# TimD1/vcfdist

Measured on AMD Instinct MI355X. Metric: supercluster-alignments/sec, higher is better.
Workload: dtype int32; 1 GPU; wgs_synth; superclusters_per_gpu=1000000, span_dist=lognormal(median 20, sigma 1.2) clip [4,10000]

## Files before the change

### vcfdist_amd/csrc/pr_zl.hip

```cpp
#ifndef PR_ZL_HIP_
#define PR_ZL_HIP_
#include <type_traits>


#define ZW_PTR(w) (int((w) & 0xffffu) - 1)
#define ZW_BASE(w) (((w) >> 16) & 0x7fu)
#define ZW_PV (1u << 23)
#define ZW_PB (1u << 24)
#define ZW_PE (1u << 25)
#define ZW_INS (1u << 26)
#define ZW_TP (1u << 27)
__device__ __forceinline__ bool zw_fwd_allow(uint32_t w) { return !(w & ZW_PV) || (w & ZW_PE); }
__device__ __forceinline__ bool zw_bwd_allow(uint32_t w) { return !(w & ZW_PV) || (w & ZW_PB); }

#define ZE_ALIVE 1u
#define ZE_HASMAT 2u
#define ZE_HASSWP 4u
#define ZE_PSLOT_SHIFT 3
#define ZE_TP 32u
#define ZE_BWD 64u

#define ZL_MAXLEN 65000
#define ZL_CLEAN_REJECT (-1)

__global__ void __launch_bounds__(256) k_prep_zl(DevBatch B, const AlnDesc *__restrict__ descs, const int32_t *__restrict__ list,
                                                 int n_list, const ZlWave *__restrict__ hdr, uint32_t *__restrict__ zin) {
    __shared__ uint32_t tile[64][65];
    __shared__ int64_t s_qo[64], s_ro[64], s_to[64];
    __shared__ int32_t s_lq[64], s_lr[64], s_lt[64];
    __shared__ uint8_t s_qs[64], s_ts[64];
    const int w = blockIdx.x;
    const ZlWave H = hdr[w];
    const int lane = threadIdx.x & 63, sub = threadIdx.x >> 6;
    if (threadIdx.x < 64) {
        const int wi = w * 64 + lane;
        const int a = wi < n_list ? list[wi] : -1;
        if (a >= 0) {
            const AlnDesc *d = descs + a;
            s_qo[lane] = d->q_off; s_ro[lane] = d->r_off; s_to[lane] = d->t_off;
            s_lq[lane] = d->Lq; s_lr[lane] = d->Lr; s_lt[lane] = d->Lt;
            s_qs[lane] = uint8_t(d->qs); s_ts[lane] = uint8_t(d->ts);
        } else {
            s_qo[lane] = s_ro[lane] = s_to[lane] = 0;
            s_lq[lane] = s_lr[lane] = s_lt[lane] = 0;
            s_qs[lane] = 0; s_ts[lane] = 2;
        }
    }
    __syncthreads();
    auto flagbits = [](int f) -> uint32_t { return ((f & PV) ? ZW_PV : 0u) | ((f & PB) ? ZW_PB : 0u) | ((f & PE) ? ZW_PE : 0u); };
    uint32_t *out = zin + H.in_off;
    for (int arr = 0; arr < 3; arr++) {
        const int mlen = arr == 0 ? H.mq : (arr == 1 ? H.mr : H.mt);
        for (int x0 = 0; x0 < mlen; x0 += 64) {
            const int x = x0 + lane;
#pragma unroll 16
            for (int k = 0; k < 16; k++) {
                const int l = sub * 16 + k;
                const int qs = s_qs[l], ts = s_ts[l];
                const int Lr = s_lr[l];
                const int len = arr == 0 ? s_lq[l] : (arr == 1 ? Lr : s_lt[l]);
                uint32_t v = 0x7f0000u;
                if (x < len) {
                    const int64_t ro = s_ro[l];
                    const int slot = arr == 2 ? ts : qs;
                    const int64_t o = (arr == 0 ? s_qo[l] : (arr == 1 ? ro : s_to[l])) + x;
                    const uint8_t *seq = arr == 1 ? B.ref_seq : B.hap_seq[slot];
                    const int2 *wk = arr == 0 ? B.wk_q[qs] : (arr == 1 ? B.wk_r[qs] : B.wk_t[ts - 2]);
                    const int2 k2 = wk[o];
                    const int p = k2.x, f = arr == 1 ? int(B.ref_flag[qs][o]) : (k2.y & 0xff);
                    const uint32_t ins = ((k2.y >> 8) & ((1 << qs) | (1 << ts))) ? ZW_INS : 0u;
                    v = uint32_t((p + 1) & 0xffff) | (uint32_t(seq[o] & 0x7f) << 16) | flagbits(f) | ins;
                    if (arr == 0 && x > 0 && ((p != wk[o - 1].x + 1) || (f & PB))) v |= ZW_TP;
                    (void)Lr;
                }
                tile[lane][l] = v;
            }
            __syncthreads();
            const int rows = min(64, mlen - x0);
            for (int r = sub; r < rows; r += 4) out[int64_t(x0 + r) * 64 + lane] = tile[r][lane];
            __syncthreads();
        }
        out += int64_t(mlen) * 64;
    }
}

typedef __attribute__((ext_vector_type(4))) unsigned int zl_u4;
typedef __attribute__((ext_vector_type(2))) unsigned int zl_u2;
#define ZL_OOB 0xfffffff0u

__global__ void __launch_bounds__(64, 6) k_zero_lane(const AlnDesc *__restrict__ descs, const int32_t *__restrict__ list, int n_list,
                                                  const ZlWave *__restrict__ hdr, const uint32_t *__restrict__ zin,
                                                  uint4 *__restrict__ zlog, AlnOut *__restrict__ outs, PathEnt *__restrict__ paths,
                                                  int keep_paths, int d1_max_rows, int prio_rows) {
    const int w = blockIdx.x, lane = threadIdx.x;
    const ZlWave H = hdr[w];
    if (H.mt >= prio_rows) __builtin_amdgcn_s_setprio(2);
    const int wi = w * 64 + lane;
    const int a_ = wi < n_list ? list[wi] : -1;
    const bool live = a_ >= 0;
    const int a = max(a_, 0);
    const AlnDesc *dp = descs + a;
    const int Lq = live ? dp->Lq : 1, Lr = live ? dp->Lr : 1, Lt = live ? dp->Lt : 0;
    const int L[2] = {Lq, Lr};
    const auto rin = __builtin_amdgcn_make_buffer_rsrc(const_cast<uint32_t *>(zin + H.in_off), 0, 256 * (H.mq + H.mr + H.mt), 0x00020000);
    const auto rlog = __builtin_amdgcn_make_buffer_rsrc(zlog + H.log_off, 0, 1280 * H.mt, 0x00020000);
    const uint32_t lane4 = uint32_t(lane) << 2, lane8 = uint32_t(lane) << 3;
    const uint32_t pos0[2] = {0u, uint32_t(H.mq) << 8}, post = uint32_t(H.mq + H.mr) << 8;
    const uint32_t logP0 = uint32_t(H.mt) << 9;
    auto in_at = [&](uint32_t off) -> uint32_t { return __builtin_amdgcn_raw_buffer_load_b32(rin, off, 0, 0); };
    bool ok = live && Lq < ZL_MAXLEN && Lr < ZL_MAXLEN && Lt < ZL_MAXLEN && Lt >= 2;
    const int rows = ok ? Lt : 0;
    int tmax = rows;
#pragma unroll
    for (int o = 32; o; o >>= 1) tmax = max(tmax, __shfl_xor(tmax, o));
    if (tmax == 0) {
        if (live) { outs[a].dist_q = D_INF; outs[a].dist_r = D_INF; outs[a].exit_min = 0; }
        return;
    }

    int qri[2][4];
    uint32_t pw[2][4];
#pragma unroll
    for (int p = 0; p < 2; p++) {
#pragma unroll
        for (int s = 0; s < 4; s++) { qri[p][s] = -1; pw[p][s] = 0; }
    }
    uint32_t tw0 = in_at(ok ? post + lane4 : ZL_OOB);
    if (ok) {
        qri[0][0] = 0; pw[0][0] = in_at(pos0[0] + lane4);
        qri[1][0] = 0; pw[1][0] = in_at(pos0[1] + lane4);
        zl_u2 e0;
        e0.x = ZE_ALIVE | ZE_HASMAT | ((pw[0][0] & ZW_TP) ? ZE_TP : 0u) | (zw_bwd_allow(pw[0][0]) ? ZE_BWD : 0u);
        e0.y = ZE_ALIVE | ZE_HASMAT | (zw_bwd_allow(pw[1][0]) ? ZE_BWD : 0u);
        __builtin_amdgcn_raw_buffer_store_b64(e0, rlog, lane8, 0, 0);
    }
    uint32_t pf_mw[2][2] = {{0, 0}, {0, 0}}, pf_sw[2][2] = {{0, 0}, {0, 0}};
    bool have_pf = false;
    auto fwd_row = [&](auto Sc, int t, bool act, uint32_t tw1) -> bool {
        constexpr int S = decltype(Sc)::value;
        const bool t_allow = zw_fwd_allow(tw0);
        uint32_t mw[2][S], sw[2][S];
        int sz[2][S];
        const bool use_pf = S == 2 && have_pf;
#pragma unroll
        for (int p = 0; p < 2; p++) {
#pragma unroll
            for (int s = 0; s < S; s++) {
                const bool alive = act && qri[p][s] >= 0;
                const int c = qri[p][s] + 1;
                const int z = ZW_PTR(pw[p][s]) + 1;
                const bool sok = alive && t_allow && zw_fwd_allow(pw[p][s]) && z < L[1 - p];
                sz[p][s] = sok ? z : -1;
                if (use_pf) {
                    mw[p][s] = (alive && c < L[p]) ? pf_mw[p][s & 1] : 0u;
                    sw[p][s] = sok ? pf_sw[p][s & 1] : 0u;
                } else {
                    mw[p][s] = in_at((alive && c < L[p]) ? pos0[p] + (uint32_t(c) << 8) + lane4 : ZL_OOB);
                    sw[p][s] = in_at(sok ? pos0[1 - p] + (uint32_t(z) << 8) + lane4 : ZL_OOB);
                }
            }
        }
        const uint32_t Tb = ZW_BASE(tw1);
        int nq[2][S];
        uint32_t nw[2][S], ne[2][S];
#pragma unroll
        for (int p = 0; p < 2; p++) {
#pragma unroll
            for (int s = 0; s < S; s++) {
                const bool hit = act && qri[p][s] >= 0 && ZW_BASE(mw[p][s]) == Tb;
                nq[p][s] = hit ? qri[p][s] + 1 : -1;
                nw[p][s] = mw[p][s];
                ne[p][s] = hit ? ZE_HASMAT : 0u;
            }
        }
        bool bad = false, full = false;
#pragma unroll
        for (int p = 0; p < 2; p++) {
            const int o = 1 - p;
#pragma unroll
            for (int s = 0; s < S; s++) {
                const bool hit = sz[p][s] >= 0 && ZW_BASE(sw[p][s]) == Tb;
                if (!__any(hit)) continue;
                const int z = sz[p][s];
                int at = -1;
#pragma unroll
                for (int k = S - 1; k >= 0; k--) at = (nq[o][k] < 0) ? k : at;
#pragma unroll
                for (int k = 0; k < S; k++) at = (nq[o][k] == z) ? k : at;
                full = full || (hit && at < 0);
#pragma unroll
                for (int k = 0; k < S; k++) {
                    const bool here = hit && at == k;
                    bad = bad || (here && (ne[o][k] & ZE_HASSWP));
                    nq[o][k] = here ? z : nq[o][k];
                    nw[o][k] = here ? sw[p][s] : nw[o][k];
                    ne[o][k] = here ? (ne[o][k] | ZE_HASSWP | (uint32_t(s) << ZE_PSLOT_SHIFT)) : ne[o][k];
                }
            }
        }
        if (S < 4 && __any(full)) return false;
        ok = ok && !bad && !full;
        if (S == 2) {
#pragma unroll
            for (int p = 0; p < 2; p++) {
#pragma unroll
                for (int s = 0; s < 2; s++) {
                    const bool alive = act && ok && nq[p][s] >= 0;
                    const int c = nq[p][s] + 1;
                    const int z = ZW_PTR(nw[p][s]) + 1;
                    pf_mw[p][s] = in_at((alive && c < L[p]) ? pos0[p] + (uint32_t(c) << 8) + lane4 : ZL_OOB);
                    pf_sw[p][s] = in_at((alive && zw_fwd_allow(nw[p][s]) && z < L[1 - p]) ? pos0[1 - p] + (uint32_t(z) << 8) + lane4 : ZL_OOB);
                }
            }
        }
        have_pf = S == 2;
        {
            zl_u2 ev;
            uint32_t wq = 0, wr_ = 0;
#pragma unroll
            for (int sl = 0; sl < S; sl++) {
                wq |= (nq[0][sl] < 0 ? 0u : (ZE_ALIVE | ne[0][sl] | ((nw[0][sl] & ZW_TP) ? ZE_TP : 0u) | (zw_bwd_allow(nw[0][sl]) ? ZE_BWD : 0u))) << (8 * sl);
                wr_ |= (nq[1][sl] < 0 ? 0u : (ZE_ALIVE | ne[1][sl] | (zw_bwd_allow(nw[1][sl]) ? ZE_BWD : 0u))) << (8 * sl);
            }
            ev.x = wq; ev.y = wr_;
            __builtin_amdgcn_raw_buffer_store_b64(ev, rlog, (act && ok) ? (uint32_t(t + 1) << 9) + lane8 : ZL_OOB, 0, 0);
        }
#pragma unroll
        for (int p = 0; p < 2; p++) {
#pragma unroll
            for (int s = 0; s < S; s++) { qri[p][s] = act ? nq[p][s] : qri[p][s]; pw[p][s] = act ? nw[p][s] : pw[p][s]; }
        }
        tw0 = act ? tw1 : tw0;
        return true;
    };
    for (int t = 0; t + 1 < tmax; t++) {
        const bool act = ok && t + 1 < rows;
        const uint32_t tw1 = in_at(act ? post + (uint32_t(t + 1) << 8) + lane4 : ZL_OOB);
        bool upper = false;
#pragma unroll
        for (int p = 0; p < 2; p++) upper = upper || (act && (qri[p][2] >= 0 || qri[p][3] >= 0));
        if (__any(upper) || !fwd_row(std::integral_constant<int, 2>{}, t, act, tw1))
            (void)fwd_row(std::integral_constant<int, 4>{}, t, act, tw1);
    }
    int endq = -1, endr = -1;
#pragma unroll
    for (int s = 0; s < 4; s++) {
        if (qri[0][s] == Lq - 1) endq = s;
        if (qri[1][s] == Lr - 1) endr = s;
    }
    const bool clean = ok && Lt <= d1_max_rows;
    ok = ok && (endq >= 0 || endr >= 0);
    if (live) {
        AlnOut &o = outs[a];
        o.dist_q = (ok && endq >= 0) ? 0 : D_INF;
        o.dist_r = (ok && endr >= 0) ? 0 : D_INF;
        o.exit_min = ok ? D_INF : (clean ? ZL_CLEAN_REJECT : 0);
    }
    if (!__any(ok)) return;

    const int nrow = ok ? Lt : 0;
    int sc[2][4];
#pragma unroll
    for (int p = 0; p < 2; p++) {
#pragma unroll
        for (int s = 0; s < 4; s++) sc[p][s] = -1;
    }
    int bmax = nrow;
#pragma unroll
    for (int o = 32; o; o >>= 1) bmax = max(bmax, __shfl_xor(bmax, o));
    auto log_row = [&](int t, bool on) -> zl_u2 {
        return __builtin_amdgcn_raw_buffer_load_b64(rlog, on ? (uint32_t(t) << 9) + lane8 : ZL_OOB, 0, 0);
    };
    zl_u2 cur = zl_u2{0, 0};
    auto bwd_row = [&](auto Sc, int t, bool act, zl_u2 pre) {
        constexpr int S = decltype(Sc)::value;
        int best[2][S];
        uint32_t pp[2][S];
#pragma unroll
        for (int p = 0; p < 2; p++) {
#pragma unroll
            for (int s = 0; s < S; s++) { best[p][s] = -1; pp[p][s] = 0; }
        }
#pragma unroll
        for (int p = 0; p < 2; p++) {
            const int o = 1 - p;
#pragma unroll
            for (int s = 0; s < S; s++) {
                const bool on = act && sc[p][s] >= 0;
                const uint32_t e = ((p ? cur.y : cur.x) >> (8 * s)) & 0xffu;
                const int tp = (e & ZE_TP) ? 1 : 0;
                {
                    const bool m = on && (e & ZE_HASMAT);
                    const int v = sc[p][s] + tp;
                    const bool gt = m && v > best[p][s], eq = m && v == best[p][s];
                    best[p][s] = gt ? v : best[p][s];
                    pp[p][s] = gt ? 1u : (eq ? (pp[p][s] | 1u) : pp[p][s]);
                }
                {
                    const bool m = on && (e & ZE_HASSWP) && (e & ZE_BWD);
                    const int v = sc[p][s] + (p == 1 ? 0 : tp);
                    const int ps = int((e >> ZE_PSLOT_SHIFT) & 3u);
                    const uint32_t mine = 2u | (uint32_t(s) << 2);
#pragma unroll
                    for (int k = 0; k < S; k++) {
                        const bool h_ = m && ps == k;
                        const bool gt = h_ && v > best[o][k], eq = h_ && v == best[o][k];
                        best[o][k] = gt ? v : best[o][k];
                        pp[o][k] = gt ? mine : (eq ? ((pp[o][k] & 1u) | mine) : pp[o][k]);
                    }
                }
            }
        }
        uint32_t ppw = 0;
#pragma unroll
        for (int p = 0; p < 2; p++) {
#pragma unroll
            for (int s = 0; s < 4; s++) {
                if (s < S) {
                    ppw |= (best[p][s] >= 0 ? pp[p][s] : 0u) << (4 * (p * 4 + s));
                    sc[p][s] = act ? best[p][s] : sc[p][s];
                } else {
                    sc[p][s] = act ? -1 : sc[p][s];
                }
            }
        }
        __builtin_amdgcn_raw_buffer_store_b32(ppw, rlog, act ? logP0 + (uint32_t(t - 1) << 8) + lane4 : ZL_OOB, 0, 0);
        if (act) cur = pre;
    };
    auto row_at = [&](int r) -> zl_u2 { return log_row(r, r >= 0 && r < nrow); };
    zl_u2 lastpre = row_at(bmax - 1);
    zl_u2 rA = row_at(bmax - 2), rB = row_at(bmax - 3), rC = row_at(bmax - 4), rD = zl_u2{0, 0};
    auto bwd_step = [&](int t, const zl_u2 &pre_reg, zl_u2 &next_reg) {
        const bool act = t >= 1 && t < nrow;
        const bool first = t == nrow - 1 && t >= 1;
        if (first) {
            const int ep = endq >= 0 ? 0 : 1, es = endq >= 0 ? endq : endr;
            cur = lastpre;
#pragma unroll
            for (int p = 0; p < 2; p++) {
#pragma unroll
                for (int s = 0; s < 4; s++) sc[p][s] = (p == ep && s == es) ? 0 : -1;
            }
        }
        next_reg = row_at(t - 4);
        const zl_u2 pre = pre_reg;
        const bool upper = act && (((cur.x | cur.y | pre.x | pre.y) & 0xffff0000u) != 0u);
        if (__any(upper)) bwd_row(std::integral_constant<int, 4>{}, t, act, pre);
        else bwd_row(std::integral_constant<int, 2>{}, t, act, pre);
        lastpre = pre;
    };
    for (int t = bmax - 1; t >= 1; t -= 4) {
        bwd_step(t, rA, rD);
        bwd_step(t - 1, rB, rA);
        bwd_step(t - 2, rC, rB);
        bwd_step(t - 3, rD, rC);
    }
    const int beg_plane = sc[0][0] >= 0 ? VPR_PLANE_QUERY : VPR_PLANE_REF;

    if (ok) outs[a].beg_plane = beg_plane;
}

struct ZlFetch {
    const uint2 *log;
    int64_t pre_i;
    uint2 pre;
    __device__ PathEnt operator()(int64_t i) {
        const uint2 v = (i == pre_i) ? pre : log[i * 64];
        if (i > 0) { pre_i = i - 1; pre = log[(i - 1) * 64]; }
        PathEnt e;
        e.a = (v.x & 0xffffu) | (((v.x >> 16) & 1u) << 31);
        e.b = uint32_t(i) | (((v.x >> 17) & 1u) << 31) | (((v.x >> 18) & 3u) << 28);
        e.qref = int(v.y & 0xffffu) - 1;
        e.tref = int(v.y >> 16) - 1;
        return e;
    }
};

__global__ void __launch_bounds__(64) k_zero_tail(DevBatch B, const AlnDesc *__restrict__ descs, const int32_t *__restrict__ list, int n_list,
                                                  const ZlWave *__restrict__ hdr, const uint32_t *__restrict__ zin,
                                                  uint4 *__restrict__ zlog, AlnOut *__restrict__ outs, PathEnt *__restrict__ paths,
                                                  int keep_paths, Section *__restrict__ secs, int32_t *const *__restrict__ fp_group,
                                                  EdJob *__restrict__ jobs, int32_t *__restrict__ n_jobs, int32_t jobs_cap, int tag,
                                                  int prio_rows) {
    const int w = blockIdx.x, lane = threadIdx.x;
    const ZlWave H = hdr[w];
    if (H.mt >= prio_rows) __builtin_amdgcn_s_setprio(2);
    const int wi = w * 64 + lane;
    const int a_ = wi < n_list ? list[wi] : -1;
    const bool live = a_ >= 0;
    const int a = max(a_, 0);
    const AlnDesc d = descs[a];
    AlnOut &O = outs[a];
    const bool ok = live && d.band_pad == tag && O.band_ok == tag;
    const int nrow = ok ? d.Lt : 0;
    int bmax = nrow;
#pragma unroll
    for (int o = 32; o; o >>= 1) bmax = max(bmax, __shfl_xor(bmax, o));
    if (bmax == 0) return;
    uint32_t status = ok ? O.status : 0u;
    bool wok = ok;
    {
        const auto rin = __builtin_amdgcn_make_buffer_rsrc(const_cast<uint32_t *>(zin + H.in_off), 0, 256 * (H.mq + H.mr + H.mt), 0x00020000);
        const auto rlog = __builtin_amdgcn_make_buffer_rsrc(zlog + H.log_off, 0, 1280 * H.mt, 0x00020000);
        const uint32_t lane4 = uint32_t(lane) << 2, lane8 = uint32_t(lane) << 3;
        const uint32_t pos0[2] = {0u, uint32_t(H.mq) << 8}, post = uint32_t(H.mq + H.mr) << 8;
        const uint32_t logP0 = uint32_t(H.mt) << 9, logS0 = logP0 + (uint32_t(H.mt) << 8);
        auto in_at = [&](uint32_t off) -> uint32_t { return __builtin_amdgcn_raw_buffer_load_b32(rin, off, 0, 0); };
        const int beg_plane = ok ? O.beg_plane : 0;
        PathEnt *path = paths + d.path_off;
        int hi = beg_plane, slot = 0, mv_in = 0, x = 0;
        uint32_t wstatus = 0;
        for (int t = 0; t < bmax; t++) {
            const bool act = wok && t < nrow;
            const uint32_t ppw = __builtin_amdgcn_raw_buffer_load_b32(rlog, (act && t + 1 < nrow) ? logP0 + (uint32_t(t) << 8) + lane4 : ZL_OOB, 0, 0);
            const uint32_t tw = in_at(act ? post + (uint32_t(t) << 8) + lane4 : ZL_OOB);
            const uint32_t cw = in_at(act ? pos0[hi] + (uint32_t(x) << 8) + lane4 : ZL_OOB);
            const int trv = ZW_PTR(tw), qref = hi ? x : ZW_PTR(cw);
            uint32_t sync = 1;
            if (mv_in) {
                const bool in_t = (tw & ZW_PV) && !(tw & ZW_PB);
                const bool in_q = hi == 0 && (cw & ZW_PV) && !(cw & ZW_PB);
                sync = (!in_t && !in_q && !((tw | cw) & ZW_INS) && trv == qref) ? 1u : 0u;
            }
            const uint32_t eqb = (ZW_BASE(cw) == ZW_BASE(tw) ? 1u : 0u) | ((hi || !(cw & ZW_PV)) ? 2u : 0u);
            zl_u2 st;
            st.x = uint32_t(x) | (uint32_t(hi) << 16) | (sync << 17) | (eqb << 18);
            st.y = uint32_t(qref + 1) | (uint32_t(trv + 1) << 16);
            __builtin_amdgcn_raw_buffer_store_b64(st, rlog, act ? logS0 + (uint32_t(t) << 9) + lane8 : ZL_OOB, 0, 0);
            if ((keep_paths & 1) && act) {
                uint4 pe;
                pe.x = uint32_t(x) | (uint32_t(hi) << 31);
                pe.y = uint32_t(t) | (sync << 31);
                pe.z = uint32_t(qref);
                pe.w = uint32_t(trv);
                *reinterpret_cast<uint4 *>(path + t) = pe;
            }
            if (act && t + 1 < nrow) {
                const uint32_t nb = (ppw >> (4 * ((hi << 2) | slot))) & 15u;
                if (hi == 1 && (nb & 2u)) { hi = 0; slot = int(nb >> 2); x = ZW_PTR(cw) + 1; }
                else if (nb & 1u) { x = x + 1; }
                else if (hi == 0 && (nb & 2u)) { hi = 1; slot = int(nb >> 2); x = ZW_PTR(cw) + 1; }
                else { wstatus |= VPR_ST_ERR_NO_PTR; wok = false; }
                mv_in = 1;
            }
        }
        if (ok) {
            O.path_len = wok ? nrow : 0;
            if (!wok) O.n_sec = 0;
            if (wstatus) atomicOr(&O.status, wstatus);
        }
        status |= wstatus;
    }
    asm volatile("s_waitcnt vmcnt(0)" ::: "memory");
    if (!ok || (status & (VPR_ST_ERR_NO_PTR | VPR_ST_ERR_LIMIT))) return;
    ZlFetch f{reinterpret_cast<const uint2 *>(zlog + H.log_off + 48 * int64_t(H.mt)) + lane, -1, make_uint2(0, 0)};
    credit_walk<false, ZlFetch, true>(B, d, O, a, nullptr, int64_t(wok ? nrow : 0), 0u, secs, fp_group, jobs, n_jobs, jobs_cap, true, f);
}

#endif
```

Baseline: 204.0 million supercluster-alignments/s.

## Software-pipeline traceback walk loads four rows ahead in zero-tail kernel

The per-row traceback walk in k_zero_tail used to issue its pointer, target and column loads for row t and then consume them immediately. It now keeps a four-deep rotating register pipeline that prefetches the loads for row t+4 and speculatively loads the next column words. When a lane switches planes, it reloads those speculative entries. The credit-walk fetcher also changes from one-ahead prefetch to batches of four log reads with a fallback load. The aim is to hide global-memory latency on this serial dependency chain, at the cost of more registers, extra loads after plane switches, and more complex control flow.

```diff
diff --git a/vcfdist_amd/csrc/pr_zl.hip b/vcfdist_amd/csrc/pr_zl.hip
--- a/vcfdist_amd/csrc/pr_zl.hip
+++ b/vcfdist_amd/csrc/pr_zl.hip
@@ -360,13 +360,30 @@
     if (ok) outs[a].beg_plane = beg_plane;
 }
 
+struct StepAhead {
+    const uint2 *log;
+    int ph;
+    int cbase;
+    uint2 c0, c1, c2, c3;
+    __device__ __forceinline__ uint2 ld(int j) const { return log[int64_t(max(j, 0)) * 64]; }
+    __device__ __forceinline__ uint2 operator()(int i) {
+        const int p = __builtin_amdgcn_readfirstlane(ph);
+        ph = (p + 1) & 3;
+        if (p == 0) { c0 = ld(i); c1 = ld(i - 1); c2 = ld(i - 2); c3 = ld(i - 3); cbase = i; }
+        const uint2 a0 = c0, a1 = c1, a2 = c2, a3 = c3;
+        const bool lo = p < 2, ev = !(p & 1);
+        uint2 v;
+        v.x = lo ? (ev ? a0.x : a1.x) : (ev ? a2.x : a3.x);
+        v.y = lo ? (ev ? a0.y : a1.y) : (ev ? a2.y : a3.y);
+        if (i != cbase - p) v = ld(i);
+        return v;
+    }
+};
+
 struct ZlFetch {
-    const uint2 *log;
-    int64_t pre_i;
-    uint2 pre;
+    StepAhead rec;
     __device__ PathEnt operator()(int64_t i) {
-        const uint2 v = (i == pre_i) ? pre : log[i * 64];
-        if (i > 0) { pre_i = i - 1; pre = log[(i - 1) * 64]; }
+        const uint2 v = rec(int(i));
         PathEnt e;
         e.a = (v.x & 0xffffu) | (((v.x >> 16) & 1u) << 31);
         e.b = uint32_t(i) | (((v.x >> 17) & 1u) << 31) | (((v.x >> 18) & 3u) << 28);
@@ -410,11 +427,18 @@
         PathEnt *path = paths + d.path_off;
         int hi = beg_plane, slot = 0, mv_in = 0, x = 0;
         uint32_t wstatus = 0;
-        for (int t = 0; t < bmax; t++) {
+        auto pp_at = [&](int t) -> uint32_t {
+            return __builtin_amdgcn_raw_buffer_load_b32(rlog, (ok && t + 1 < nrow) ? logP0 + (uint32_t(t) << 8) + lane4 : ZL_OOB, 0, 0);
+        };
+        auto tw_at = [&](int t) -> uint32_t { return in_at((ok && t < nrow) ? post + (uint32_t(t) << 8) + lane4 : ZL_OOB); };
+        auto cw_at = [&](int p, int xx, bool on) -> uint32_t { return in_at(on ? pos0[p] + (uint32_t(xx) << 8) + lane4 : ZL_OOB); };
+        uint32_t pA = pp_at(0), tA = tw_at(0), cA = cw_at(hi, 0, ok);
+        uint32_t pB = pp_at(1), tB = tw_at(1), cB = cw_at(hi, 1, ok);
+        uint32_t pC = pp_at(2), tC = tw_at(2), cC = cw_at(hi, 2, ok);
+        uint32_t pD = pp_at(3), tD = tw_at(3), cD = cw_at(hi, 3, ok);
+        auto walk_row = [&](int t, uint32_t &pK, uint32_t &tK, uint32_t &cK, uint32_t &c1, uint32_t &c2, uint32_t &c3) {
             const bool act = wok && t < nrow;
-            const uint32_t ppw = __builtin_amdgcn_raw_buffer_load_b32(rlog, (act && t + 1 < nrow) ? logP0 + (uint32_t(t) << 8) + lane4 : ZL_OOB, 0, 0);
-            const uint32_t tw = in_at(act ? post + (uint32_t(t) << 8) + lane4 : ZL_OOB);
-            const uint32_t cw = in_at(act ? pos0[hi] + (uint32_t(x) << 8) + lane4 : ZL_OOB);
+            const uint32_t ppw = pK, tw = tK, cw = cK;
             const int trv = ZW_PTR(tw), qref = hi ? x : ZW_PTR(cw);
             uint32_t sync = 1;
             if (mv_in) {
@@ -435,14 +459,30 @@
                 pe.w = uint32_t(trv);
                 *reinterpret_cast<uint4 *>(path + t) = pe;
             }
+            bool swp = false;
             if (act && t + 1 < nrow) {
                 const uint32_t nb = (ppw >> (4 * ((hi << 2) | slot))) & 15u;
-                if (hi == 1 && (nb & 2u)) { hi = 0; slot = int(nb >> 2); x = ZW_PTR(cw) + 1; }
+                if (hi == 1 && (nb & 2u)) { hi = 0; slot = int(nb >> 2); x = ZW_PTR(cw) + 1; swp = true; }
                 else if (nb & 1u) { x = x + 1; }
-                else if (hi == 0 && (nb & 2u)) { hi = 1; slot = int(nb >> 2); x = ZW_PTR(cw) + 1; }
+                else if (hi == 0 && (nb & 2u)) { hi = 1; slot = int(nb >> 2); x = ZW_PTR(cw) + 1; swp = true; }
                 else { wstatus |= VPR_ST_ERR_NO_PTR; wok = false; }
                 mv_in = 1;
             }
+            pK = pp_at(t + 4);
+            tK = tw_at(t + 4);
+            cK = cw_at(hi, x + 3, ok && t + 4 < nrow);
+            if (__any(swp)) {
+                const uint32_t n1 = cw_at(hi, x, swp), n2 = cw_at(hi, x + 1, swp), n3 = cw_at(hi, x + 2, swp);
+                c1 = swp ? n1 : c1;
+                c2 = swp ? n2 : c2;
+                c3 = swp ? n3 : c3;
+            }
+        };
+        for (int t = 0; t < bmax; t += 4) {
+            walk_row(t, pA, tA, cA, cB, cC, cD);
+            walk_row(t + 1, pB, tB, cB, cC, cD, cA);
+            walk_row(t + 2, pC, tC, cC, cD, cA, cB);
+            walk_row(t + 3, pD, tD, cD, cA, cB, cC);
         }
         if (ok) {
             O.path_len = wok ? nrow : 0;
@@ -453,7 +493,7 @@
     }
     asm volatile("s_waitcnt vmcnt(0)" ::: "memory");
     if (!ok || (status & (VPR_ST_ERR_NO_PTR | VPR_ST_ERR_LIMIT))) return;
-    ZlFetch f{reinterpret_cast<const uint2 *>(zlog + H.log_off + 48 * int64_t(H.mt)) + lane, -1, make_uint2(0, 0)};
+    ZlFetch f{{reinterpret_cast<const uint2 *>(zlog + H.log_off + 48 * int64_t(H.mt)) + lane, 0, -8, {0, 0}, {0, 0}, {0, 0}, {0, 0}}};
     credit_walk<false, ZlFetch, true>(B, d, O, a, nullptr, int64_t(wok ? nrow : 0), 0u, secs, fp_group, jobs, n_jobs, jobs_cap, true, f);
 }
 
```

Result: slower. 199.7 million supercluster-alignments/s (-2.1%).
